# zju-vipa/ProtoPFormer

Measured on AMD Instinct MI355X. Metric: images/sec train step, deit_small+2000 protos, bs256, 1/2/4/8 MI355X, higher is better.
Workload: dtype bf16; 1 GPU; deit_small_patch16_224, synthetic 224x224, 2000x384 prototypes, 200 classes, k=81, batch 256/GPU (BASELINE.json configs[2]), train step = fwd+CE+PPC+bwd+allreduce+AdamW+EMA, DropPath 0.1; blocks after the token reservation run compacted on the 1+k reserved rows (equal to the masked full-length blocks to bf16 rounding); bf16 backbone: the reserved tokens differ from the fp32 reference's in ~2-3 % o; global_batch=256, parallelism=dp1

## Files before the change

### include/ppf_hip.h

```cpp
#ifndef PPF_HIP_H
#define PPF_HIP_H

#include <stddef.h>
#include <stdint.h>

#ifdef __cplusplus
extern "C" {
#endif

typedef struct ihipStream_t* ppf_stream_t;

#define PPF_ERR_SHAPE (-1)
#define PPF_ERR_ALIGN (-2)
#define PPF_ERR_ARG (-3)

#define PPF_ABI_VERSION 10

const char* ppf_last_error(void);
int ppf_abi_version(void);
int ppf_device_info(int* cu_count, int* clock_mhz, char* name, int name_len);
int ppf_stream_arm(ppf_stream_t stream, int on);
int ppf_stream_wait_stream(ppf_stream_t dst, ppf_stream_t src);
int64_t ppf_stream_mark(ppf_stream_t stream);
int ppf_stream_wait_mark(ppf_stream_t stream, int64_t ticket);
// ... 159 lines not shown
                        ppf_stream_t stream);
int ppf_assemble_tokens_bwd(const float* dx, void* dtok, float* dpos, float* dcls, int B, int Np, int D, int lead,
                            ppf_stream_t stream);
int ppf_sigmoid_bwd_blocks(int rows);
int ppf_sigmoid_bwd(const float* df, const float* f, void* dz, float* dbias, int rows, int cols, float* partial, size_t partial_bytes,
                    ppf_stream_t stream);
int ppf_adamw_step(float* p, const float* g, float* m, float* v, float* ema, void* p16, int64_t n, int nseg,
                   const int64_t* seg_bounds, const float* seg_lr, const float* seg_wd, float beta1, float beta2, float eps,
                   int step, float ema_decay, float grad_scale, ppf_stream_t stream);
int ppf_adamw_step_dev(float* p, const float* g, float* m, float* v, float* ema, void* p16, int64_t n, int nseg,
                       const int64_t* seg_bounds, const float* hyper, float beta1, float beta2, float eps, float ema_decay,
                       ppf_stream_t stream);
int ppf_adamw_step_guarded(float* p, const float* g, float* m, float* v, float* ema, void* p16, int64_t n, int nseg,
                           const int64_t* seg_bounds, const float* hyper, float beta1, float beta2, float eps, float ema_decay,
                           const float* loss, int* nonfinite_flag, ppf_stream_t stream);
int ppf_hyper_set(float* hyper, const float* host_vals, int n, ppf_stream_t stream);
int ppf_clip_grad_blocks(void);
int ppf_clip_grad_scale(const float* g, int64_t n, float max_norm, float pre_scale, float* partial, float* hyper, float* norm_out,
                        ppf_stream_t stream);
int ppf_droppath_scales(float* out, const float* keep, int nslot, int B, uint64_t seed, void* state_u64, ppf_stream_t stream);
int ppf_reserved_rows_map(const int* idx, int* rows, int B, int k, int N, ppf_stream_t stream);
int ppf_gather_rows(const void* src, const int* rows, void* dst, int nrows, int row_bytes, ppf_stream_t stream);
int ppf_scatter_rows(const void* src, const int* rows, void* dst, int nrows_src, int nrows_dst, int row_bytes, ppf_stream_t stream);
int ppf_memset_zero(void* ptr, size_t bytes, ppf_stream_t stream);
int ppf_copy_2d(void* dst, int64_t dst_pitch, const void* src, int64_t src_pitch, int64_t width, int64_t rows, ppf_stream_t stream);
int ppf_image_finish_u8(const void* in_u8_hwc, float* out_nchw, int B, int H, int W, const float* mean3, const float* std3,
                        const int* rects, uint64_t seed, const void* state_u64, ppf_stream_t stream);
#define PPF_MIX_KIND 0
#define PPF_MIX_YL 1
#define PPF_MIX_YH 2
#define PPF_MIX_XL 3
#define PPF_MIX_XH 4
#define PPF_MIX_WSELF 5
#define PPF_MIX_WOTHER 6
#define PPF_MIX_WORDS 8
int ppf_mixup_apply(float* x, const int* table_host, int* table_dev, int B, int Cc, int H, int W, ppf_stream_t stream);
int ppf_mixup_target(const void* label_i64, const float* lam, int lam_stride, float off_value, float on_value, float* target, int B,
                     int C, ppf_stream_t stream);
int ppf_scale_by_scalar(const float* x, const float* scalar_dev, float* out, int64_t n, ppf_stream_t stream);

int ppf_im2col_patch_f32(const float* img, float* cols, int B, int C, int H, int W, int patch, ppf_stream_t stream);
int ppf_layernorm_fwd_f32(const float* x, const int* row_map, const float* w, const float* b, float* y, int rows, int D, float eps,
                          ppf_stream_t stream);
int ppf_epilogue_f32(float* C, const float* bias, int kind, const float* res, const float* rowscale, int rows_per_group,
                     const float* colscale, int M, int N, ppf_stream_t stream);
int ppf_attn_fwd_f32(const float* qkv, float* out, const float* policy, float* headmean, int NP, int B, int H, int N, int D,
// ... 11 lines not shown
```

### protopformer_amd/backbone.py

```python
import functools
import os

import torch
import torch.nn as nn

from . import _lib, ops
from .ops import EPI_ATOMIC, EPI_BF16, EPI_DGELU, EPI_F32, EPI_GELU, EPI_RESID, EPI_SIGMOID_F32

LN_EPS = 1e-6
_KEEP_CACHE = {}
_ROW_BWD_MAX_ELEMS = 12_000_000


def _row_bwd(M, D):
    return M * D <= _ROW_BWD_MAX_ELEMS


def droppath_scales(rates, B, device, training):
    slots = [r if training else 0.0 for r in rates]
    active = [i for i, r in enumerate(slots) if r > 0.0]
    if not active:
        return None, [-1] * len(slots)
    key = (tuple(slots), str(device))
    st = _KEEP_CACHE.get(key)
# ... 391 lines not shown
    dnf = head_bwd(ppnet, store, saved, df)
    alloc = ops.zeros if head["row_map"] is not None else (lambda shape, dtype, device: torch.empty(shape, dtype=dtype, device=device))
    dx = alloc((M, D), torch.float32, dev)
    dyb = lane.track(alloc((M, D), torch.bfloat16, dev))
    last = feats.blocks[-1]
    lnb(dnf, x_last.reshape(M, D), feats.norm.weight, head["meanf"], head["rstdf"], store.grad_view(feats.norm.weight),
        store.grad_view(feats.norm.bias), dx_out=dx, row_map=head["row_map"], cast_out=dyb, rowscale=layers[-1]["s2"],
        rows_per_group=N, dbias_next=store.grad_view(last.mlp.fc2.bias))
    gs = getattr(ppnet, "_grad_sync", None)
    if gs is not None:
        chunk_ready(gs, lane, gs.tail_chunk)
    bwd = functools.partial(block_bwd, next_dyb=dyb_ring(lane, D), lnb=lnb, dgrad=functools.partial(_dgrad, store),
                            attn_bwd=lambda blk, L, dao: ops.attn_bwd(L["qkv"], L["ao"], dao, L["rowmax"], L["zinv"], B, feats.num_heads, L["N"], D,
                                                                      policy=L["policy"], self_keep=True, eps_n=L["eps_n"]))
    bias_done = True
    for i in range(len(layers) - 1, -1, -1):
        L = layers[i]
        Nl = L["N"]
        row_tile = row_tile_bwd(store, feats.blocks[i], D, ops.rowgemm_tile_rows(B * Nl, Nl, backward=True)) if _row_bwd(B * Nl, D) else None
        dyb, bias_done = bwd(feats.blocks[i], store, L, dx, dyb, bias_done, (feats.blocks[i - 1], layers[i - 1]) if i > 0 else None,
                             row_tile=row_tile)
        if i > 0 and L["rows"] is not None:
            Mf = B * layers[i - 1]["N"]
            dx = ops.scatter_rows(dx, L["rows"], Mf)
            dyb = lane.track(ops.scatter_rows(dyb, L["rows"], Mf))
        if gs is not None and i in gs.block_chunk:
            chunk_ready(gs, lane, gs.block_chunk[i])
    if layers and layers[0]["rows"] is not None:
        dx = ops.scatter_rows(dx, layers[0]["rows"], B * (feats.patch_embed.num_patches + 1))
    return embed_bwd(ppnet, store, saved, dx, 1)


class TokensFn(torch.autograd.Function):

    @staticmethod
    def forward(ctx, img, ppnet, dp, *params):
        store = ppnet.flat_store()
        store.refresh_bf16()
        feats = ppnet.features
        need_bwd = any(ctx.needs_input_grad)
        if need_bwd and "t16_params" in ppnet._arch_fns:
            if store._t16 is None:
                store.register_transposed(ppnet._arch_fns["t16_params"](feats))
            if store._t16 is not None and not store._t16["fresh"] and feats.embed_dim <= 256:
                wgrad_lane(store).submit(store.refresh_t16, (store.bf16, store._t16["buf"]), defer=True)
            else:
                store.refresh_t16()
        saved = {} if need_bwd else None
        (layer, k), = ppnet.reserve_layer_nums
        fwd = ppnet._arch_fns
        x = fwd["embed"](feats, store, img, saved)
        x_out, cls_attn, idx, layers = fwd["blocks"](feats, store, x, layer, k, dp, save=need_bwd)
# ... 27 lines not shown
```

### protopformer_amd/csrc/elementwise.hip

```cpp
#include "ppf_common.h"
#include "ppf_hip.h"

namespace {

__global__ __launch_bounds__(256) void cast_kernel(const float* __restrict__ in, bf16_t* __restrict__ out, int64_t n8) {
    for (int64_t i = (int64_t)blockIdx.x * 256 + threadIdx.x; i < n8; i += (int64_t)gridDim.x * 256) {
        const float4 a = reinterpret_cast<const float4*>(in)[2 * i], b = reinterpret_cast<const float4*>(in)[2 * i + 1];
        reinterpret_cast<uint4*>(out)[i] = make_uint4(pack_bf16x2(a.x, a.y), pack_bf16x2(a.z, a.w), pack_bf16x2(b.x, b.y), pack_bf16x2(b.z, b.w));
    }
}

__global__ __launch_bounds__(256) void widen_kernel(const bf16_t* __restrict__ in, float* __restrict__ out, int64_t n8) {
    for (int64_t i = (int64_t)blockIdx.x * 256 + threadIdx.x; i < n8; i += (int64_t)gridDim.x * 256) {
        const uint4 u = reinterpret_cast<const uint4*>(in)[i];
        const float2 a = unpack_bf16x2(u.x), b = unpack_bf16x2(u.y), c = unpack_bf16x2(u.z), d = unpack_bf16x2(u.w);
        reinterpret_cast<float4*>(out)[2 * i] = make_float4(a.x, a.y, b.x, b.y);
        reinterpret_cast<float4*>(out)[2 * i + 1] = make_float4(c.x, c.y, d.x, d.y);
    }
}

__global__ __launch_bounds__(256) void im2col_kernel(const float* __restrict__ img, bf16_t* __restrict__ cols, int B, int C,
                                                     int H, int W, int p, int64_t total8) {
    const int gh = H / p, gw = W / p, pp8 = p / 8, kdim = C * p * p;
    for (int64_t i = (int64_t)blockIdx.x * 256 + threadIdx.x; i < total8; i += (int64_t)gridDim.x * 256) {
// ... 192 lines not shown
                out[i] = floorf(kp + u) / kp;
            }
        }
    }
    __syncthreads();
    if (threadIdx.x == 0) state[0] = step + 1;
}

__global__ __launch_bounds__(256) void rows_map_kernel(const int* __restrict__ idx, int* __restrict__ rows, int B, int k, int N) {
    const int i = blockIdx.x * 256 + threadIdx.x;
    if (i >= B * (k + 1)) return;
    const int b = i / (k + 1), j = i % (k + 1);
    rows[i] = b * N + (j == 0 ? 0 : 1 + idx[b * k + j - 1]);
}
__global__ __launch_bounds__(256) void move_rows_kernel(const uint4* __restrict__ src, const int* __restrict__ rows, uint4* __restrict__ dst,
                                                        int nrows, int vec, int scatter) {
    const int64_t total = (int64_t)nrows * vec;
    for (int64_t i = (int64_t)blockIdx.x * 256 + threadIdx.x; i < total; i += (int64_t)gridDim.x * 256) {
        const int r = (int)(i / vec), c = (int)(i % vec);
        const int64_t o = (int64_t)rows[r] * vec + c;
        if (scatter) dst[o] = src[i]; else dst[i] = src[o];
    }
}
__global__ __launch_bounds__(256) void scale_by_kernel(const float* __restrict__ x, const float* __restrict__ scalar, float* __restrict__ out, int64_t n) {
    const float s = *scalar;
    for (int64_t i = (int64_t)blockIdx.x * 256 + threadIdx.x; i < n; i += (int64_t)gridDim.x * 256) out[i] = x[i] * s;
}

struct FinishParams { const unsigned char* in; float* out; const int* rects; int B, H, W; float mean[3], inv_std[3]; uint64_t seed; const unsigned long long* state; };
__global__ __launch_bounds__(256) void image_finish_kernel(const FinishParams p) {
    const int64_t hw = (int64_t)p.H * p.W, total4 = (int64_t)p.B * hw / 4;
    const unsigned long long step = p.state ? p.state[0] : 0ull;
    for (int64_t i = (int64_t)blockIdx.x * 256 + threadIdx.x; i < total4; i += (int64_t)gridDim.x * 256) {
        const int b = (int)((i * 4) / hw);
        const int64_t pix = i * 4 - (int64_t)b * hw;
        const int y = (int)(pix / p.W), x = (int)(pix % p.W);
        const unsigned char* src = p.in + ((int64_t)b * hw + pix) * 3;
        const uint32_t w0 = reinterpret_cast<const uint32_t*>(src)[0], w1 = reinterpret_cast<const uint32_t*>(src)[1], w2 = reinterpret_cast<const uint32_t*>(src)[2];
        const unsigned char px[12] = {(unsigned char)w0, (unsigned char)(w0 >> 8), (unsigned char)(w0 >> 16), (unsigned char)(w0 >> 24),
                                      (unsigned char)w1, (unsigned char)(w1 >> 8), (unsigned char)(w1 >> 16), (unsigned char)(w1 >> 24),
                                      (unsigned char)w2, (unsigned char)(w2 >> 8), (unsigned char)(w2 >> 16), (unsigned char)(w2 >> 24)};
        int ry = 0, rx = 0, rh = 0, rw = 0;
        if (p.rects) { ry = p.rects[4 * b]; rx = p.rects[4 * b + 1]; rh = p.rects[4 * b + 2]; rw = p.rects[4 * b + 3]; }
        const bool row_in = rh > 0 && y >= ry && y < ry + rh;
#pragma unroll
        for (int c = 0; c < 3; ++c) {
// ... 170 lines not shown
    PPF_CHECK_ARG(nslot > 0 && B > 0 && out && keep && state_u64, PPF_ERR_ARG, "ppf_droppath_scales: bad arguments");
    return ppf_launch<droppath_kernel>(dim3(1), dim3(256), 0, stream, "ppf_droppath_scales", out, keep, nslot, B, seed, (unsigned long long*)state_u64);
}

int ppf_reserved_rows_map(const int* idx, int* rows, int B, int k, int N, hipStream_t stream) {
    PPF_CHECK_ARG(B > 0 && k > 0 && N > k, PPF_ERR_SHAPE, "ppf_reserved_rows_map: bad shape B=%d k=%d N=%d", B, k, N);
    return ppf_launch<rows_map_kernel>(dim3((B * (k + 1) + 255) / 256), dim3(256), 0, stream, "ppf_reserved_rows_map", idx, rows, B, k, N);
}

int ppf_gather_rows(const void* src, const int* rows, void* dst, int nrows, int row_bytes, hipStream_t stream) {
    PPF_CHECK_ARG(nrows > 0 && row_bytes > 0 && row_bytes % 16 == 0, PPF_ERR_ALIGN, "ppf_gather_rows: row_bytes=%d must be a positive multiple of 16", row_bytes);
    return ppf_launch<move_rows_kernel>(dim3(grid_for((int64_t)nrows * (row_bytes / 16))), dim3(256), 0, stream, "ppf_gather_rows", (const uint4*)src, rows,
                                        (uint4*)dst, nrows, row_bytes / 16, 0);
}

int ppf_scatter_rows(const void* src, const int* rows, void* dst, int nrows_src, int nrows_dst, int row_bytes, hipStream_t stream) {
    PPF_CHECK_ARG(nrows_src > 0 && nrows_dst >= nrows_src && row_bytes > 0 && row_bytes % 16 == 0, PPF_ERR_ALIGN, "ppf_scatter_rows: bad arguments");
    hipError_t e = ppf_memset_async(dst, 0, (size_t)nrows_dst * row_bytes, stream);
    if (e != hipSuccess) { ppf_set_error("ppf_scatter_rows: memset failed: %s", hipGetErrorString(e)); return (int)e; }
    return ppf_launch<move_rows_kernel>(dim3(grid_for((int64_t)nrows_src * (row_bytes / 16))), dim3(256), 0, stream, "ppf_scatter_rows", (const uint4*)src, rows,
                                        (uint4*)dst, nrows_src, row_bytes / 16, 1);
}

int ppf_image_finish_u8(const void* in_u8_hwc, float* out_nchw, int B, int H, int W, const float* mean3, const float* std3, const int* rects,
                        uint64_t seed, const void* state_u64, hipStream_t stream) {
    PPF_CHECK_ARG(B > 0 && H > 0 && W > 0 && W % 4 == 0 && in_u8_hwc && out_nchw && mean3 && std3, PPF_ERR_ARG, "ppf_image_finish_u8: bad arguments (W %% 4 == 0)");
    PPF_CHECK_ARG((((uintptr_t)in_u8_hwc) & 3) == 0 && (((uintptr_t)out_nchw) & 15) == 0, PPF_ERR_ALIGN, "ppf_image_finish_u8: alignment");
    FinishParams p;
    p.in = (const unsigned char*)in_u8_hwc; p.out = out_nchw; p.rects = rects; p.B = B; p.H = H; p.W = W; p.seed = seed;
    p.state = (const unsigned long long*)state_u64;
    for (int c = 0; c < 3; ++c) { p.mean[c] = mean3[c]; p.inv_std[c] = 1.0f / std3[c]; }
    return ppf_launch<image_finish_kernel>(dim3(grid_for((int64_t)B * H * W / 4)), dim3(256), 0, stream, "ppf_image_finish_u8", p);
}

int ppf_memset_zero(void* ptr, size_t bytes, hipStream_t stream) {
    if (bytes == 0) return 0;
    hipError_t e = ppf_memset_async(ptr, 0, bytes, stream);
    if (e != hipSuccess) { ppf_set_error("ppf_memset_zero: %s", hipGetErrorString(e)); return (int)e; }
    return 0;
}

int ppf_scale_by_scalar(const float* x, const float* scalar_dev, float* out, int64_t n, hipStream_t stream) {
    PPF_CHECK_ARG(n > 0 && x && scalar_dev && out, PPF_ERR_ARG, "ppf_scale_by_scalar: bad arguments");
    return ppf_launch<scale_by_kernel>(dim3(grid_for(n)), dim3(256), 0, stream, "ppf_scale_by_scalar", x, scalar_dev, out, n);
}

// ... 19 lines not shown
```

### protopformer_amd/csrc/head.hip

```cpp
#include "ppf_common.h"
#include "ppf_hip.h"
#include "ppf_select.h"

namespace {

constexpr int MAXPPC = 16;

struct PpcParams {
    const float* act;
    const int* idx;
    const long long* label;
    int B, P, T, ppc, side;
    float cov_thresh, mean_thresh;
    float* partial;
    float* gcov;
    float* gmean;
};

__global__ __launch_bounds__(256) void ppc_kernel(const PpcParams p) {
    __shared__ float mu[MAXPPC][2], S[MAXPPC], hinge_cov[MAXPPC], gmu[MAXPPC][2];
    __shared__ float mean_sum;
    const int lane = threadIdx.x & 63, wave = threadIdx.x >> 6, b = blockIdx.x;
    const int N = p.side * p.side;
    const float nfac = (float)N / (float)(N - 1);
    const int lab = (int)p.label[b];
    const float inv_cnt = 1.0f / ((float)p.B * (float)p.ppc);
    for (int j = wave; j < p.ppc; j += 4) {
        const float* w = p.act + ((size_t)b * p.P + (size_t)lab * p.ppc + j) * p.T;
        float s = 0.f, sx = 0.f, sy = 0.f;
        for (int t = lane; t < p.T; t += 64) {
            const int id = p.idx[(size_t)b * p.T + t];
            const float wt = w[t], x = (float)(id / p.side), y = (float)(id % p.side);
            s += wt; sx += wt * x; sy += wt * y;
        }
        s = wave_sum(s); sx = wave_sum(sx); sy = wave_sum(sy);
        const float mx = sx / s, my = sy / s;
        float v = 0.f;
        for (int t = lane; t < p.T; t += 64) {
            const int id = p.idx[(size_t)b * p.T + t];
            const float dx = (float)(id / p.side) - mx, dy = (float)(id % p.side) - my;
            v += w[t] * (dx * dx + dy * dy);
        }
        v = wave_sum(v) / s;
        const float c = 0.5f * nfac * v;
        const bool on = c > p.cov_thresh;
        for (int t = lane; t < p.T; t += 64) {
            const int id = p.idx[(size_t)b * p.T + t];
            const float dx = (float)(id / p.side) - mx, dy = (float)(id % p.side) - my;
            p.gcov[((size_t)b * p.ppc + j) * p.T + t] = on ? inv_cnt * 0.5f * nfac * ((dx * dx + dy * dy) - v) / s : 0.f;
        }
        if (lane == 0) { mu[j][0] = mx; mu[j][1] = my; S[j] = s; hinge_cov[j] = on ? c - p.cov_thresh : 0.f; }
    }
    __syncthreads();
    if (threadIdx.x == 0) {
        float ms = 0.f;
        for (int j = 0; j < p.ppc; ++j) { gmu[j][0] = 0.f; gmu[j][1] = 0.f; }
        const float pair_norm = 1.0f / ((float)p.B * (float)p.ppc * (float)p.ppc);
        for (int j = 0; j < p.ppc; ++j)
            for (int k = 0; k < p.ppc; ++k) {
                if (j == k) continue;
                const float dx = mu[j][0] - mu[k][0], dy = mu[j][1] - mu[k][1];
                const float d = sqrtf(dx * dx + dy * dy);
                if (p.mean_thresh - d > 0.f) {
                    ms += p.mean_thresh - d;
                    if (d > 0.f) {
                        gmu[j][0] -= 2.0f * pair_norm * dx / d;
                        gmu[j][1] -= 2.0f * pair_norm * dy / d;
                    }
                }
            }
        mean_sum = ms;
        float cs = 0.f;
        for (int j = 0; j < p.ppc; ++j) cs += hinge_cov[j];
        p.partial[2 * b] = cs;
        p.partial[2 * b + 1] = ms;
    }
    __syncthreads();
    for (int j = wave; j < p.ppc; j += 4) {
        const float mx = mu[j][0], my = mu[j][1], s = S[j], gx = gmu[j][0], gy = gmu[j][1];
        for (int t = lane; t < p.T; t += 64) {
            const int id = p.idx[(size_t)b * p.T + t];
            const float dx = (float)(id / p.side) - mx, dy = (float)(id % p.side) - my;
            p.gmean[((size_t)b * p.ppc + j) * p.T + t] = (gx * dx + gy * dy) / s;
        }
    }
}

__global__ __launch_bounds__(256) void reduce_cols_kernel(const float* in, int n, int stride, int cols, float s0, float s1, float* out) {
    __shared__ float red[256];
    for (int c = 0; c < cols; ++c) {
        float s = 0.f;
        for (int i = threadIdx.x; i < n; i += 256) s += in[(size_t)i * stride + c];
        red[threadIdx.x] = s;
        __syncthreads();
        for (int o = 128; o > 0; o >>= 1) {
            if (threadIdx.x < o) red[threadIdx.x] += red[threadIdx.x + o];
            __syncthreads();
        }
        if (threadIdx.x == 0) out[c] = red[0] * (c == 0 ? s0 : s1);
        __syncthreads();
    }
}

__global__ __launch_bounds__(256) void ppc_bwd_kernel(const float* gcov, const float* gmean, const float* up_cov, const float* up_mean,
                                                      const long long* label, float* g_full, int B, int P, int T, int ppc) {
    const int b = blockIdx.x;
    const float uc = up_cov ? up_cov[0] : 0.f, um = up_mean ? up_mean[0] : 0.f;
    const int lab = (int)label[b];
    for (int i = threadIdx.x; i < ppc * T; i += 256) {
        const int j = i / T, t = i % T;
        g_full[((size_t)b * P + (size_t)lab * ppc + j) * T + t] = uc * gcov[((size_t)b * ppc + j) * T + t] + um * gmean[((size_t)b * ppc + j) * T + t];
    }
}

__global__ __launch_bounds__(256) void ce_kernel(const float* logits, const long long* label, float* per_sample, float* dlogits, int B, int C) {
    const int lane = threadIdx.x & 63, wave = threadIdx.x >> 6;
    const int b = blockIdx.x * 4 + wave;
    if (b >= B) return;
    const float* row = logits + (size_t)b * C;
    float mx = -INFINITY;
    for (int c = lane; c < C; c += 64) mx = fmaxf(mx, row[c]);
    mx = wave_max(mx);
    float s = 0.f;
    for (int c = lane; c < C; c += 64) s += __expf(row[c] - mx);
    s = wave_sum(s);
    const int lab = (int)label[b];
    const float lse = mx + __logf(s);
    if (lane == 0) per_sample[b] = lse - row[lab];
    const float invB = 1.0f / (float)B;
    for (int c = lane; c < C; c += 64) dlogits[(size_t)b * C + c] = (__expf(row[c] - lse) - (c == lab ? 1.0f : 0.0f)) * invB;
}

__global__ __launch_bounds__(256) void soft_ce_kernel(const float* logits, const float* target, const long long* label, float smoothing,
                                                      float* per_sample, float* dlogits, int B, int C) {
    const int lane = threadIdx.x & 63, wave = threadIdx.x >> 6;
    const int b = blockIdx.x * 4 + wave;
    if (b >= B) return;
    const float* row = logits + (size_t)b * C;
    float mxf = -INFINITY;
    for (int c = lane; c < C; c += 64) mxf = fmaxf(mxf, row[c]);
    const double mx = (double)wave_max(mxf);
    double s = 0.0;
    for (int c = lane; c < C; c += 64) s += exp((double)row[c] - mx);
    const double ls = log(wave_sum_f64(s));
    const double invB = 1.0 / (double)B;
    if (target) {
        const float* t = target + (size_t)b * C;
        double st = 0.0, acc = 0.0;
        for (int c = lane; c < C; c += 64) {
            const double tc = (double)t[c];
            st += tc;
            acc += tc * ((mx - (double)row[c]) + ls);
        }
        st = wave_sum_f64(st);
        acc = wave_sum_f64(acc);
        if (lane == 0) per_sample[b] = (float)acc;
        for (int c = lane; c < C; c += 64)
            dlogits[(size_t)b * C + c] = (float)((exp((double)row[c] - mx - ls) * st - (double)t[c]) * invB);
    } else {
        const long long lab = label[b];
        double dlab = 0.0, dsum = 0.0;
        for (int c = lane; c < C; c += 64) {
            const double d = mx - (double)row[c];
            dsum += d;
            if (c == lab) dlab = d;
        }
        dlab = wave_sum_f64(dlab);
        dsum = wave_sum_f64(dsum);
        const double sm = (double)smoothing, conf = 1.0 - sm, off = sm / (double)C;
        if (lane == 0) per_sample[b] = (float)(conf * (dlab + ls) + sm * (dsum / (double)C + ls));
        for (int c = lane; c < C; c += 64)
            dlogits[(size_t)b * C + c] = (float)((exp((double)row[c] - mx - ls) - (c == lab ? conf : 0.0) - off) * invB);
    }
}

constexpr int EVAL_MAX_WG = 1024, EVAL_NV = 6;
__device__ double g_eval_partial[EVAL_MAX_WG * EVAL_NV];

__device__ __forceinline__ int wave_argmax_first(const float* row, int C, int lane, float& mx_out) {
    float mx = -INFINITY;
    int at = 0x7fffffff;
    for (int c = lane; c < C; c += 64) {
        const float x = row[c];
        if (x > mx || at == 0x7fffffff) { mx = x; at = c; }
    }
    wave_first(mx, at);
    mx_out = mx;
    return at;
}

__global__ __launch_bounds__(256) void eval_metrics_kernel(const float* __restrict__ logits, const float* __restrict__ logits_global,
                                                           const float* __restrict__ logits_local, const long long* __restrict__ label,
                                                           int B, int C) {
    __shared__ double red[4][EVAL_NV];
    const int lane = threadIdx.x & 63, wave = threadIdx.x >> 6;
    double ce = 0.0;
// ... 213 lines not shown
    float p0 = 0.f, p1 = 0.f;
    if (n < q0.N) { for (int z = 0; z < q0.S; ++z) p0 += part[q0.part_off + ((size_t)z * M + m) * q0.N + n]; if (q0.out) q0.out[(size_t)m * q0.ldo + n] = q0.alpha * p0; }
    if (n < q1.N) { for (int z = 0; z < q1.S; ++z) p1 += part[q1.part_off + ((size_t)z * M + m) * q1.N + n]; if (q1.out) q1.out[(size_t)m * q1.ldo + n] = q1.alpha * p1; }
    if (sum) sum[(size_t)m * ldsum + n] = q0.c * p0 + q1.c * p1;
}

__global__ __launch_bounds__(256) void axpbypcz_kernel(const float* x, const float* y, const float* z, float* out, float a, float b, float c, int64_t n) {
    for (int64_t i = (int64_t)blockIdx.x * 256 + threadIdx.x; i < n; i += (int64_t)gridDim.x * 256) out[i] = a * x[i] + b * y[i] + c * z[i];
}
__global__ __launch_bounds__(256) void axpby_kernel(const float* x, const float* y, float* out, float a, float b, int64_t n) {
    for (int64_t i = (int64_t)blockIdx.x * 256 + threadIdx.x; i < n; i += (int64_t)gridDim.x * 256) out[i] = a * x[i] + b * y[i];
}

}

extern "C" {

int ppf_ppc_loss(const float* act, const int* idx, const void* label, int B, int P, int T, int ppc, int side, float cov_thresh,
                 float mean_thresh, float* partial, float* gcov, float* gmean, float* loss, hipStream_t stream) {
    PPF_CHECK_ARG(B > 0 && P > 0 && T > 0 && ppc >= 1 && ppc <= MAXPPC && side >= 2 && P % ppc == 0, PPF_ERR_SHAPE, "ppf_ppc_loss: bad shape");
    PpcParams p;
    p.act = act; p.idx = idx; p.label = (const long long*)label; p.B = B; p.P = P; p.T = T; p.ppc = ppc; p.side = side;
    p.cov_thresh = cov_thresh; p.mean_thresh = mean_thresh; p.partial = partial; p.gcov = gcov; p.gmean = gmean;
    if (int rc = ppf_launch<ppc_kernel>(dim3(B), dim3(256), 0, stream, "ppf_ppc_loss", p)) return rc;
    return ppf_launch<reduce_cols_kernel>(dim3(1), dim3(256), 0, stream, "ppf_ppc_loss", partial, B, 2, 2, 1.0f / ((float)B * ppc), 1.0f / ((float)B * ppc * ppc), loss);
}

int ppf_ppc_loss_bwd(const float* gcov, const float* gmean, const float* up_cov, const float* up_mean, const void* label, float* g_full, int B,
                     int P, int T, int ppc, hipStream_t stream) {
    PPF_CHECK_ARG(B > 0 && P > 0 && T > 0 && ppc >= 1, PPF_ERR_SHAPE, "ppf_ppc_loss_bwd: bad shape");
    return ppf_launch<ppc_bwd_kernel>(dim3(B), dim3(256), 0, stream, "ppf_ppc_loss_bwd", gcov, gmean, up_cov, up_mean, (const long long*)label, g_full, B, P, T, ppc);
}

int ppf_cross_entropy(const float* logits, const void* label, float* per_sample, float* dlogits, float* loss, int B, int C, hipStream_t stream) {
    PPF_CHECK_ARG(B > 0 && C > 0, PPF_ERR_SHAPE, "ppf_cross_entropy: bad shape");
    if (int rc = ppf_launch<ce_kernel>(dim3((B + 3) / 4), dim3(256), 0, stream, "ppf_cross_entropy", logits, (const long long*)label, per_sample, dlogits, B, C)) return rc;
    return ppf_launch<reduce_cols_kernel>(dim3(1), dim3(256), 0, stream, "ppf_cross_entropy", per_sample, B, 1, 1, 1.0f / (float)B, 0.f, loss);
}

int ppf_soft_cross_entropy(const float* logits, const float* target, const void* label, float smoothing, float* per_sample, float* dlogits,
                           float* loss, int B, int C, hipStream_t stream) {
    PPF_CHECK_ARG(B > 0 && C > 0, PPF_ERR_SHAPE, "ppf_soft_cross_entropy: bad shape B=%d C=%d", B, C);
    PPF_CHECK_ARG(logits && per_sample && dlogits && loss, PPF_ERR_ARG, "ppf_soft_cross_entropy: null pointer");
    PPF_CHECK_ARG((target == nullptr) != (label == nullptr), PPF_ERR_ARG, "ppf_soft_cross_entropy: pass exactly one of target / label");
    PPF_CHECK_ARG(target || (smoothing >= 0.f && smoothing <= 1.f), PPF_ERR_ARG, "ppf_soft_cross_entropy: smoothing %g outside [0, 1]",
                  (double)smoothing);
    if (int rc = ppf_launch<soft_ce_kernel>(dim3((B + 3) / 4), dim3(256), 0, stream, "ppf_soft_cross_entropy", logits, target, (const long long*)label, smoothing,
                                            per_sample, dlogits, B, C)) return rc;
    return ppf_launch<reduce_cols_kernel>(dim3(1), dim3(256), 0, stream, "ppf_soft_cross_entropy", per_sample, B, 1, 1, 1.0f / (float)B, 0.f, loss);
}

int ppf_eval_metrics(const float* logits, const float* logits_global, const float* logits_local, const void* label, double* acc, int B, int C,
                     hipStream_t stream) {
    PPF_CHECK_ARG(B > 0 && C > 0, PPF_ERR_SHAPE, "ppf_eval_metrics: bad shape B=%d C=%d", B, C);
    PPF_CHECK_ARG(logits && label && acc, PPF_ERR_ARG, "ppf_eval_metrics: null pointer");
    const int nwg = (B + 3) / 4 < EVAL_MAX_WG ? (B + 3) / 4 : EVAL_MAX_WG;
    if (int rc = ppf_launch<eval_metrics_kernel>(dim3(nwg), dim3(256), 0, stream, "ppf_eval_metrics", logits, logits_global, logits_local, (const long long*)label, B, C)) return rc;
    return ppf_launch<eval_metrics_finish_kernel>(dim3(1), dim3(256), 0, stream, "ppf_eval_metrics", acc, nwg, B, logits_global != nullptr, logits_local != nullptr);
}

int ppf_sgemm(const float* A, const float* Bm, float* C, int M, int N, int K, int64_t sam, int64_t sak, int64_t sbn, int64_t sbk, int ldc,
              float alpha, float beta, float* workspace, int64_t workspace_floats, hipStream_t stream) {
    PPF_CHECK_ARG(M > 0 && N > 0 && K > 0, PPF_ERR_SHAPE, "ppf_sgemm: bad shape");
    int S = workspace ? (int)(workspace_floats / ((int64_t)M * N)) : 1;
    if (S > 16) S = 16;
    if (S > (K + 127) / 128) S = (K + 127) / 128;
    if (S < 1) S = 1;
    const int kchunk = ((K + S - 1) / S + 31) / 32 * 32;
    S = (K + kchunk - 1) / kchunk;
    int rc;
    if ((int64_t)M * N * K >= (int64_t(1) << 28) && M >= 64 && N >= 64) {
        const int tiles = ((N + SM_T - 1) / SM_T) * ((M + SM_T - 1) / SM_T);
// ... 50 lines not shown
```

### protopformer_amd/csrc/ppf_runtime.hip

```cpp
#include "ppf_common.h"
#include "ppf_hip.h"
#include <cstdarg>
#include <cstdio>
#include <cstdlib>

static thread_local char g_err[512] = "";

extern "C" {

void ppf_set_error(const char* fmt, ...) {
    va_list ap;
    va_start(ap, fmt);
    vsnprintf(g_err, sizeof(g_err), fmt, ap);
    va_end(ap);
}

const char* ppf_last_error(void) { return g_err; }

int ppf_abi_version(void) { return PPF_ABI_VERSION; }

int ppf_device_info(int* cu_count, int* clock_mhz, char* name, int name_len) {
    hipDeviceProp_t prop;
    int dev = 0;
    hipError_t e = hipGetDevice(&dev);
// ... 61 lines not shown
    hipError_t e = hipStreamWaitEvent(stream, ring_event(ticket), 0);
    if (e != hipSuccess) { ppf_set_error("ppf_stream_wait_mark: %s", hipGetErrorString(e)); return (int)e; }
    return 0;
}

namespace {
PpfEventPool g_path[PPF_PROBE_NTAGS];
constexpr size_t PATH_PROBE_CAP = 4096;
bool g_path_on = false;
}

}

hipEvent_t ppf_take_stop_event(hipStream_t s) {
    for (auto& a : g_arm)
        if (a.used && a.armed && a.s == s) { a.ev = ring_event(g_seq++); a.have = true; return a.ev; }
    return nullptr;
}
void ppf_note_enqueue(hipStream_t s) {
    for (auto& a : g_arm)
        if (a.used && a.s == s) a.have = false;
}

int ppf_cu_count() {
    static const int cus = [] {
        int dev = 0, n = 256;
        (void)hipGetDevice(&dev);
        (void)hipDeviceGetAttribute(&n, hipDeviceAttributeMultiprocessorCount, dev);
        return n > 0 ? n : 256;
    }();
    return cus;
}

std::pair<hipEvent_t, hipEvent_t> PpfEventPool::acquire() {
    if (used == pool.size()) {
        hipEvent_t a = nullptr, b = nullptr;
        (void)hipEventCreateWithFlags(&a, hipEventDisableSystemFence); (void)hipEventCreateWithFlags(&b, hipEventDisableSystemFence);
        pool.emplace_back(a, b);
    }
    return pool[used++];
}
void PpfEventPool::reset() { used = 0; flops = 0.0; bytes = 0.0; }
void PpfEventPool::destroy() {
    for (auto& e : pool) { (void)hipEventDestroy(e.first); (void)hipEventDestroy(e.second); }
    pool.clear(); used = 0;
}
// ... 47 lines not shown
```

### protopformer_amd/ops.py

```python
import torch

from . import _lib

EPI_BF16, EPI_F32, EPI_GELU, EPI_SIGMOID_F32, EPI_RESID, EPI_DGELU, EPI_ATOMIC = range(7)


DOMINANT_NAME = ("weight-gradient bf16 MFMA GEMM, split over the contraction, ordered partial tiles: wgrad8_kernel<4,2> / <2,4> (256x128 / 128x256 tiles) "
                 "and gemm_kernel<TA=1,TB=1,EPI_PARTIAL,COLSUM> (128x128)")


_WORKSPACE = {}
_GEMM_WS = {}
_RETIRED_WS = []


def _workspace(device, nbytes, pool=_WORKSPACE):
    key = (device, _lib.stream_ptr())
    buf = pool.get(key)
    if buf is None or buf.numel() < nbytes:
        if buf is not None:
            _RETIRED_WS.append(buf)
        buf = torch.empty(max(nbytes, 64 << 20), dtype=torch.uint8, device=device)
        pool[key] = buf
    return buf
# ... 845 lines not shown
def cat_rows(first, rest):
    B, N, D = rest.shape
    out = torch.empty((B, N + 1, D), dtype=rest.dtype, device=rest.device)
    o2 = out.reshape(B, (N + 1) * D)
    copy_2d(o2[:, :D], first.reshape(B, D))
    copy_2d(o2[:, D:], rest.reshape(B, N * D))
    return out


def reserved_rows_map(idx, N):
    B, k = idx.shape
    rows = torch.empty(B * (k + 1), dtype=torch.int32, device=idx.device)
    _lib.call("ppf_reserved_rows_map", idx, rows, B, k, N)
    return rows


def gather_rows(src, rows):
    _chk(src)
    dst = torch.empty((rows.numel(), src.shape[1]), dtype=src.dtype, device=src.device)
    _lib.call("ppf_gather_rows", src, rows, dst, rows.numel(), src.shape[1] * src.element_size())
    return dst


def scatter_rows(src, rows, nrows_dst):
    _chk(src)
    dst = torch.empty((nrows_dst, src.shape[1]), dtype=src.dtype, device=src.device)
    _lib.call("ppf_scatter_rows", src, rows, dst, src.shape[0], nrows_dst, src.shape[1] * src.element_size())
    return dst


def droppath_draw(out, keep, seed, state):
    nslot, B = out.shape
    _lib.call("ppf_droppath_scales", out, keep, nslot, B, int(seed) & 0xFFFFFFFFFFFFFFFF, state)
    return out


def scale_by_scalar(x, scalar):
    out = torch.empty_like(x)
    _lib.call("ppf_scale_by_scalar", x, scalar, out, x.numel())
    return out


def th_fused_ok(H, N, D):
    return bool(_lib.lib().ppf_th_fused_supported(H, N, D))


def th_fwd(qkv, wl, bl, ww, bw, hm_out, B, H, N, D):
    NP, NPK = (N + 3) // 4 * 4, (N + 7) // 8 * 8
    a16 = torch.empty((B, H, N, NPK), dtype=torch.bfloat16, device=qkv.device)
    rowmax = torch.empty((B, H, N), dtype=torch.float32, device=qkv.device)
# ... 159 lines not shown
```

Baseline: 17320 images/sec.

## Fuse loss reductions into kernels via last-block finish; grouped row scatter

The cross-entropy, soft cross-entropy and PPC loss kernels now do their own final reduction. The last workgroup to arrive on a per-stream atomic counter reduces the partials, which removes the separate one-block reduce_cols launch after each. The PPC kernel also moves to 1024 threads. Backward row scatter switches to a per-sample grouped kernel that builds an inverse map in LDS and writes each destination row once, copied or zeroed, with nontemporal stores. This is meant to avoid a separate zero-fill-plus-scatter pass. The cost is atomic counter state tied to a stream slot table, and reliance on correct fence ordering.

```diff
diff --git a/include/ppf_hip.h b/include/ppf_hip.h
--- a/include/ppf_hip.h
+++ b/include/ppf_hip.h
@@ -205,6 +205,8 @@
 int ppf_reserved_rows_map(const int* idx, int* rows, int B, int k, int N, ppf_stream_t stream);
 int ppf_gather_rows(const void* src, const int* rows, void* dst, int nrows, int row_bytes, ppf_stream_t stream);
 int ppf_scatter_rows(const void* src, const int* rows, void* dst, int nrows_src, int nrows_dst, int row_bytes, ppf_stream_t stream);
+int ppf_scatter_rows_grouped(const void* src, const int* rows, void* dst, int groups, int rows_per_group_src, int rows_per_group_dst,
+                             int row_bytes, ppf_stream_t stream);
 int ppf_memset_zero(void* ptr, size_t bytes, ppf_stream_t stream);
 int ppf_copy_2d(void* dst, int64_t dst_pitch, const void* src, int64_t src_pitch, int64_t width, int64_t rows, ppf_stream_t stream);
 int ppf_image_finish_u8(const void* in_u8_hwc, float* out_nchw, int B, int H, int W, const float* mean3, const float* std3,
diff --git a/protopformer_amd/backbone.py b/protopformer_amd/backbone.py
--- a/protopformer_amd/backbone.py
+++ b/protopformer_amd/backbone.py
@@ -437,12 +437,12 @@
                              row_tile=row_tile)
         if i > 0 and L["rows"] is not None:
             Mf = B * layers[i - 1]["N"]
-            dx = ops.scatter_rows(dx, L["rows"], Mf)
-            dyb = lane.track(ops.scatter_rows(dyb, L["rows"], Mf))
+            dx = ops.scatter_rows(dx, L["rows"], Mf, groups=B)
+            dyb = lane.track(ops.scatter_rows(dyb, L["rows"], Mf, groups=B))
         if gs is not None and i in gs.block_chunk:
             chunk_ready(gs, lane, gs.block_chunk[i])
     if layers and layers[0]["rows"] is not None:
-        dx = ops.scatter_rows(dx, layers[0]["rows"], B * (feats.patch_embed.num_patches + 1))
+        dx = ops.scatter_rows(dx, layers[0]["rows"], B * (feats.patch_embed.num_patches + 1), groups=B)
     return embed_bwd(ppnet, store, saved, dx, 1)
 
 
diff --git a/protopformer_amd/csrc/elementwise.hip b/protopformer_amd/csrc/elementwise.hip
--- a/protopformer_amd/csrc/elementwise.hip
+++ b/protopformer_amd/csrc/elementwise.hip
@@ -238,6 +238,32 @@
         if (scatter) dst[o] = src[i]; else dst[i] = src[o];
     }
 }
+__global__ __launch_bounds__(256) void scatter_rows_grouped_kernel(const uint4* __restrict__ src, const int* __restrict__ rows, uint4* __restrict__ dst,
+                                                                   int ns, int nd, int vec) {
+    extern __shared__ int inv[];
+    const int b = blockIdx.x;
+    for (int d = threadIdx.x; d < nd; d += 256) inv[d] = -1;
+    __syncthreads();
+    for (int j = threadIdx.x; j < ns; j += 256) {
+        const int d = rows[(size_t)b * ns + j] - b * nd;
+        if (d >= 0 && d < nd) inv[d] = j;
+    }
+    __syncthreads();
+    typedef unsigned int u32x4 __attribute__((ext_vector_type(4)));
+    const int per = (nd + gridDim.y - 1) / gridDim.y, d0 = blockIdx.y * per, d1 = min(nd, d0 + per);
+    const int lane = threadIdx.x & 63;
+    for (int d = d0 + (threadIdx.x >> 6); d < d1; d += 4) {
+        const int j = inv[d];
+        u32x4* o = reinterpret_cast<u32x4*>(dst + ((size_t)b * nd + d) * vec);
+        if (j >= 0) {
+            const u32x4* s = reinterpret_cast<const u32x4*>(src + ((size_t)b * ns + j) * vec);
+            for (int c = lane; c < vec; c += 64) __builtin_nontemporal_store(s[c], o + c);
+        } else {
+            const u32x4 zero = {0u, 0u, 0u, 0u};
+            for (int c = lane; c < vec; c += 64) __builtin_nontemporal_store(zero, o + c);
+        }
+    }
+}
 __global__ __launch_bounds__(256) void scale_by_kernel(const float* __restrict__ x, const float* __restrict__ scalar, float* __restrict__ out, int64_t n) {
     const float s = *scalar;
     for (int64_t i = (int64_t)blockIdx.x * 256 + threadIdx.x; i < n; i += (int64_t)gridDim.x * 256) out[i] = x[i] * s;
@@ -454,6 +480,22 @@
                                         (uint4*)dst, nrows_src, row_bytes / 16, 1);
 }
 
+int ppf_scatter_rows_grouped(const void* src, const int* rows, void* dst, int groups, int rows_per_group_src, int rows_per_group_dst, int row_bytes,
+                             hipStream_t stream) {
+    PPF_CHECK_ARG(src && rows && dst && groups > 0 && rows_per_group_src > 0 && rows_per_group_dst >= rows_per_group_src, PPF_ERR_SHAPE,
+                  "ppf_scatter_rows_grouped: bad shape groups=%d rows %d -> %d", groups, rows_per_group_src, rows_per_group_dst);
+    PPF_CHECK_ARG(row_bytes > 0 && row_bytes % 16 == 0 && ((uintptr_t)src & 15) == 0 && ((uintptr_t)dst & 15) == 0, PPF_ERR_ALIGN,
+                  "ppf_scatter_rows_grouped: row_bytes=%d and both pointers must be multiples of 16", row_bytes);
+    PPF_CHECK_ARG(rows_per_group_dst <= 16000 && groups <= 0x7fffffff / rows_per_group_dst,
+                  PPF_ERR_SHAPE, "ppf_scatter_rows_grouped: group of %d rows too large (inverse table in LDS: <= 16000 rows)", rows_per_group_dst);
+    int split = (8 * ppf_cu_count() + groups - 1) / groups;
+    if (split > rows_per_group_dst) split = rows_per_group_dst;
+    if (split > 65535) split = 65535;
+    if (split < 1) split = 1;
+    return ppf_launch<scatter_rows_grouped_kernel>(dim3(groups, split), dim3(256), (size_t)rows_per_group_dst * sizeof(int), stream, "ppf_scatter_rows_grouped",
+                                                   (const uint4*)src, rows, (uint4*)dst, rows_per_group_src, rows_per_group_dst, row_bytes / 16);
+}
+
 int ppf_image_finish_u8(const void* in_u8_hwc, float* out_nchw, int B, int H, int W, const float* mean3, const float* std3, const int* rects,
                         uint64_t seed, const void* state_u64, hipStream_t stream) {
     PPF_CHECK_ARG(B > 0 && H > 0 && W > 0 && W % 4 == 0 && in_u8_hwc && out_nchw && mean3 && std3, PPF_ERR_ARG, "ppf_image_finish_u8: bad arguments (W %% 4 == 0)");
diff --git a/protopformer_amd/csrc/head.hip b/protopformer_amd/csrc/head.hip
--- a/protopformer_amd/csrc/head.hip
+++ b/protopformer_amd/csrc/head.hip
@@ -1,4 +1,5 @@
 #include "ppf_common.h"
+#include "ppf_finish.h"
 #include "ppf_hip.h"
 #include "ppf_select.h"
 
@@ -15,17 +16,42 @@
     float* partial;
     float* gcov;
     float* gmean;
+    float* loss;
+    float s_cov, s_mean;
+    int slot;
 };
 
-__global__ __launch_bounds__(256) void ppc_kernel(const PpcParams p) {
+enum { FIN_CE = 0, FIN_SOFT_CE = 1, FIN_PPC = 2, FIN_SCALARS = 4 };
+__device__ unsigned g_fin_scalar[PPF_FINISH_STREAMS][FIN_SCALARS];
+
+__device__ __forceinline__ void reduce_cols(float* red, const float* in, int n, int stride, int cols, float s0, float s1, float* out) {
+    for (int c = 0; c < cols; ++c) {
+        if (threadIdx.x < 256) {
+            float s = 0.f;
+            for (int i = threadIdx.x; i < n; i += 256) s += in[(size_t)i * stride + c];
+            red[threadIdx.x] = s;
+        }
+        __syncthreads();
+        for (int o = 128; o > 0; o >>= 1) {
+            if (threadIdx.x < o) red[threadIdx.x] += red[threadIdx.x + o];
+            __syncthreads();
+        }
+        if (threadIdx.x == 0) out[c] = red[0] * (c == 0 ? s0 : s1);
+        __syncthreads();
+    }
+}
+
+constexpr int PPC_THREADS = 1024;
+__global__ __launch_bounds__(PPC_THREADS) void ppc_kernel(const PpcParams p) {
     __shared__ float mu[MAXPPC][2], S[MAXPPC], hinge_cov[MAXPPC], gmu[MAXPPC][2];
     __shared__ float mean_sum;
+    __shared__ float red[256];
     const int lane = threadIdx.x & 63, wave = threadIdx.x >> 6, b = blockIdx.x;
     const int N = p.side * p.side;
     const float nfac = (float)N / (float)(N - 1);
     const int lab = (int)p.label[b];
     const float inv_cnt = 1.0f / ((float)p.B * (float)p.ppc);
-    for (int j = wave; j < p.ppc; j += 4) {
+    for (int j = wave; j < p.ppc; j += PPC_THREADS / 64) {
         const float* w = p.act + ((size_t)b * p.P + (size_t)lab * p.ppc + j) * p.T;
         float s = 0.f, sx = 0.f, sy = 0.f;
         for (int t = lane; t < p.T; t += 64) {
@@ -72,11 +98,11 @@
         mean_sum = ms;
         float cs = 0.f;
         for (int j = 0; j < p.ppc; ++j) cs += hinge_cov[j];
-        p.partial[2 * b] = cs;
-        p.partial[2 * b + 1] = ms;
+        ppf_finish_store(p.partial + 2 * b, cs);
+        ppf_finish_store(p.partial + 2 * b + 1, ms);
     }
     __syncthreads();
-    for (int j = wave; j < p.ppc; j += 4) {
+    for (int j = wave; j < p.ppc; j += PPC_THREADS / 64) {
         const float mx = mu[j][0], my = mu[j][1], s = S[j], gx = gmu[j][0], gy = gmu[j][1];
         for (int t = lane; t < p.T; t += 64) {
             const int id = p.idx[(size_t)b * p.T + t];
@@ -84,22 +110,8 @@
             p.gmean[((size_t)b * p.ppc + j) * p.T + t] = (gx * dx + gy * dy) / s;
         }
     }
-}
-
-__global__ __launch_bounds__(256) void reduce_cols_kernel(const float* in, int n, int stride, int cols, float s0, float s1, float* out) {
-    __shared__ float red[256];
-    for (int c = 0; c < cols; ++c) {
-        float s = 0.f;
-        for (int i = threadIdx.x; i < n; i += 256) s += in[(size_t)i * stride + c];
-        red[threadIdx.x] = s;
-        __syncthreads();
-        for (int o = 128; o > 0; o >>= 1) {
-            if (threadIdx.x < o) red[threadIdx.x] += red[threadIdx.x + o];
-            __syncthreads();
-        }
-        if (threadIdx.x == 0) out[c] = red[0] * (c == 0 ? s0 : s1);
-        __syncthreads();
-    }
+    if (ppf_finish_arrive(&g_fin_scalar[p.slot][FIN_PPC], gridDim.x, reinterpret_cast<unsigned*>(red)))
+        reduce_cols(red, p.partial, p.B, 2, 2, p.s_cov, p.s_mean, p.loss);
 }
 
 __global__ __launch_bounds__(256) void ppc_bwd_kernel(const float* gcov, const float* gmean, const float* up_cov, const float* up_mean,
@@ -113,29 +125,31 @@
     }
 }
 
-__global__ __launch_bounds__(256) void ce_kernel(const float* logits, const long long* label, float* per_sample, float* dlogits, int B, int C) {
+__global__ __launch_bounds__(256) void ce_kernel(const float* logits, const long long* label, float* per_sample, float* dlogits, float* loss,
+                                                 int B, int C, int slot) {
+    __shared__ float red[256];
     const int lane = threadIdx.x & 63, wave = threadIdx.x >> 6;
     const int b = blockIdx.x * 4 + wave;
-    if (b >= B) return;
-    const float* row = logits + (size_t)b * C;
-    float mx = -INFINITY;
-    for (int c = lane; c < C; c += 64) mx = fmaxf(mx, row[c]);
-    mx = wave_max(mx);
-    float s = 0.f;
-    for (int c = lane; c < C; c += 64) s += __expf(row[c] - mx);
-    s = wave_sum(s);
-    const int lab = (int)label[b];
-    const float lse = mx + __logf(s);
-    if (lane == 0) per_sample[b] = lse - row[lab];
-    const float invB = 1.0f / (float)B;
-    for (int c = lane; c < C; c += 64) dlogits[(size_t)b * C + c] = (__expf(row[c] - lse) - (c == lab ? 1.0f : 0.0f)) * invB;
-}
-
-__global__ __launch_bounds__(256) void soft_ce_kernel(const float* logits, const float* target, const long long* label, float smoothing,
-                                                      float* per_sample, float* dlogits, int B, int C) {
-    const int lane = threadIdx.x & 63, wave = threadIdx.x >> 6;
-    const int b = blockIdx.x * 4 + wave;
-    if (b >= B) return;
+    if (b < B) {
+        const float* row = logits + (size_t)b * C;
+        float mx = -INFINITY;
+        for (int c = lane; c < C; c += 64) mx = fmaxf(mx, row[c]);
+        mx = wave_max(mx);
+        float s = 0.f;
+        for (int c = lane; c < C; c += 64) s += __expf(row[c] - mx);
+        s = wave_sum(s);
+        const int lab = (int)label[b];
+        const float lse = mx + __logf(s);
+        if (lane == 0) ppf_finish_store(per_sample + b, lse - row[lab]);
+        const float invB = 1.0f / (float)B;
+        for (int c = lane; c < C; c += 64) dlogits[(size_t)b * C + c] = (__expf(row[c] - lse) - (c == lab ? 1.0f : 0.0f)) * invB;
+    }
+    if (ppf_finish_arrive(&g_fin_scalar[slot][FIN_CE], gridDim.x, reinterpret_cast<unsigned*>(red)))
+        reduce_cols(red, per_sample, B, 1, 1, 1.0f / (float)B, 0.f, loss);
+}
+
+__device__ __forceinline__ void soft_ce_row(const float* logits, const float* target, const long long* label, float smoothing, float* per_sample,
+                                            float* dlogits, int B, int C, int b, int lane) {
     const float* row = logits + (size_t)b * C;
     float mxf = -INFINITY;
     for (int c = lane; c < C; c += 64) mxf = fmaxf(mxf, row[c]);
@@ -154,7 +168,7 @@
         }
         st = wave_sum_f64(st);
         acc = wave_sum_f64(acc);
-        if (lane == 0) per_sample[b] = (float)acc;
+        if (lane == 0) ppf_finish_store(per_sample + b, (float)acc);
         for (int c = lane; c < C; c += 64)
             dlogits[(size_t)b * C + c] = (float)((exp((double)row[c] - mx - ls) * st - (double)t[c]) * invB);
     } else {
@@ -168,10 +182,19 @@
         dlab = wave_sum_f64(dlab);
         dsum = wave_sum_f64(dsum);
         const double sm = (double)smoothing, conf = 1.0 - sm, off = sm / (double)C;
-        if (lane == 0) per_sample[b] = (float)(conf * (dlab + ls) + sm * (dsum / (double)C + ls));
+        if (lane == 0) ppf_finish_store(per_sample + b, (float)(conf * (dlab + ls) + sm * (dsum / (double)C + ls)));
         for (int c = lane; c < C; c += 64)
             dlogits[(size_t)b * C + c] = (float)((exp((double)row[c] - mx - ls) - (c == lab ? conf : 0.0) - off) * invB);
     }
+}
+__global__ __launch_bounds__(256) void soft_ce_kernel(const float* logits, const float* target, const long long* label, float smoothing,
+                                                      float* per_sample, float* dlogits, float* loss, int B, int C, int slot) {
+    __shared__ float red[256];
+    const int lane = threadIdx.x & 63, wave = threadIdx.x >> 6;
+    const int b = blockIdx.x * 4 + wave;
+    if (b < B) soft_ce_row(logits, target, label, smoothing, per_sample, dlogits, B, C, b, lane);
+    if (ppf_finish_arrive(&g_fin_scalar[slot][FIN_SOFT_CE], gridDim.x, reinterpret_cast<unsigned*>(red)))
+        reduce_cols(red, per_sample, B, 1, 1, 1.0f / (float)B, 0.f, loss);
 }
 
 constexpr int EVAL_MAX_WG = 1024, EVAL_NV = 6;
@@ -431,8 +454,9 @@
     PpcParams p;
     p.act = act; p.idx = idx; p.label = (const long long*)label; p.B = B; p.P = P; p.T = T; p.ppc = ppc; p.side = side;
     p.cov_thresh = cov_thresh; p.mean_thresh = mean_thresh; p.partial = partial; p.gcov = gcov; p.gmean = gmean;
-    if (int rc = ppf_launch<ppc_kernel>(dim3(B), dim3(256), 0, stream, "ppf_ppc_loss", p)) return rc;
-    return ppf_launch<reduce_cols_kernel>(dim3(1), dim3(256), 0, stream, "ppf_ppc_loss", partial, B, 2, 2, 1.0f / ((float)B * ppc), 1.0f / ((float)B * ppc * ppc), loss);
+    p.loss = loss; p.s_cov = 1.0f / ((float)B * ppc); p.s_mean = 1.0f / ((float)B * ppc * ppc);
+    if ((p.slot = ppf_finish_slot(stream, "ppf_ppc_loss")) < 0) return PPF_ERR_ARG;
+    return ppf_launch<ppc_kernel>(dim3(B), dim3(PPC_THREADS), 0, stream, "ppf_ppc_loss", p);
 }
 
 int ppf_ppc_loss_bwd(const float* gcov, const float* gmean, const float* up_cov, const float* up_mean, const void* label, float* g_full, int B,
@@ -443,8 +467,9 @@
 
 int ppf_cross_entropy(const float* logits, const void* label, float* per_sample, float* dlogits, float* loss, int B, int C, hipStream_t stream) {
     PPF_CHECK_ARG(B > 0 && C > 0, PPF_ERR_SHAPE, "ppf_cross_entropy: bad shape");
-    if (int rc = ppf_launch<ce_kernel>(dim3((B + 3) / 4), dim3(256), 0, stream, "ppf_cross_entropy", logits, (const long long*)label, per_sample, dlogits, B, C)) return rc;
-    return ppf_launch<reduce_cols_kernel>(dim3(1), dim3(256), 0, stream, "ppf_cross_entropy", per_sample, B, 1, 1, 1.0f / (float)B, 0.f, loss);
+    const int slot = ppf_finish_slot(stream, "ppf_cross_entropy");
+    if (slot < 0) return PPF_ERR_ARG;
+    return ppf_launch<ce_kernel>(dim3((B + 3) / 4), dim3(256), 0, stream, "ppf_cross_entropy", logits, (const long long*)label, per_sample, dlogits, loss, B, C, slot);
 }
 
 int ppf_soft_cross_entropy(const float* logits, const float* target, const void* label, float smoothing, float* per_sample, float* dlogits,
@@ -454,9 +479,10 @@
     PPF_CHECK_ARG((target == nullptr) != (label == nullptr), PPF_ERR_ARG, "ppf_soft_cross_entropy: pass exactly one of target / label");
     PPF_CHECK_ARG(target || (smoothing >= 0.f && smoothing <= 1.f), PPF_ERR_ARG, "ppf_soft_cross_entropy: smoothing %g outside [0, 1]",
                   (double)smoothing);
-    if (int rc = ppf_launch<soft_ce_kernel>(dim3((B + 3) / 4), dim3(256), 0, stream, "ppf_soft_cross_entropy", logits, target, (const long long*)label, smoothing,
-                                            per_sample, dlogits, B, C)) return rc;
-    return ppf_launch<reduce_cols_kernel>(dim3(1), dim3(256), 0, stream, "ppf_soft_cross_entropy", per_sample, B, 1, 1, 1.0f / (float)B, 0.f, loss);
+    const int slot = ppf_finish_slot(stream, "ppf_soft_cross_entropy");
+    if (slot < 0) return PPF_ERR_ARG;
+    return ppf_launch<soft_ce_kernel>(dim3((B + 3) / 4), dim3(256), 0, stream, "ppf_soft_cross_entropy", logits, target, (const long long*)label, smoothing,
+                                      per_sample, dlogits, loss, B, C, slot);
 }
 
 int ppf_eval_metrics(const float* logits, const float* logits_global, const float* logits_local, const void* label, double* acc, int B, int C,
diff --git a/protopformer_amd/csrc/ppf_finish.h b/protopformer_amd/csrc/ppf_finish.h
--- /dev/null
+++ b/protopformer_amd/csrc/ppf_finish.h
@@ -0,0 +1,27 @@
+#pragma once
+#include "ppf_common.h"
+
+constexpr int PPF_FINISH_STREAMS = 64;
+
+__attribute__((visibility("hidden"))) int ppf_finish_slot(hipStream_t stream, const char* who);
+
+__device__ __forceinline__ void ppf_finish_store(float* p, float v) { __hip_atomic_store(p, v, __ATOMIC_RELAXED, __HIP_MEMORY_SCOPE_AGENT); }
+
+__device__ __forceinline__ bool ppf_finish_arrive(unsigned* counter, unsigned n, unsigned* lds_word) {
+    asm volatile("s_waitcnt vmcnt(0)" ::: "memory");
+    __syncthreads();
+    if (threadIdx.x == 0) {
+        const unsigned old = __hip_atomic_fetch_add(counter, 1u, __ATOMIC_RELAXED, __HIP_MEMORY_SCOPE_AGENT);
+        const bool last = old + 1u == n;
+        if (last) {
+            __hip_atomic_store(counter, 0u, __ATOMIC_RELAXED, __HIP_MEMORY_SCOPE_AGENT);
+            __builtin_amdgcn_fence(__ATOMIC_ACQUIRE, "agent");
+            asm volatile("s_waitcnt vmcnt(0)" ::: "memory");
+        }
+        *lds_word = last ? 1u : 0u;
+    }
+    __syncthreads();
+    const bool mine = *lds_word != 0u;
+    __syncthreads();
+    return mine;
+}
diff --git a/protopformer_amd/csrc/ppf_runtime.hip b/protopformer_amd/csrc/ppf_runtime.hip
--- a/protopformer_amd/csrc/ppf_runtime.hip
+++ b/protopformer_amd/csrc/ppf_runtime.hip
@@ -1,4 +1,5 @@
 #include "ppf_common.h"
+#include "ppf_finish.h"
 #include "ppf_hip.h"
 #include <cstdarg>
 #include <cstdio>
@@ -107,6 +108,19 @@
         if (a.used && a.s == s) a.have = false;
 }
 
+int ppf_finish_slot(hipStream_t stream, const char* who) {
+    static hipStream_t table[PPF_FINISH_STREAMS];
+    static int used = 0;
+    for (int i = 0; i < used; ++i)
+        if (table[i] == stream) return i;
+    if (used == PPF_FINISH_STREAMS) {
+        ppf_set_error("%s: more than %d streams have used the in-launch reductions of this process", who, PPF_FINISH_STREAMS);
+        return -1;
+    }
+    table[used] = stream;
+    return used++;
+}
+
 int ppf_cu_count() {
     static const int cus = [] {
         int dev = 0, n = 256;
diff --git a/protopformer_amd/ops.py b/protopformer_amd/ops.py
--- a/protopformer_amd/ops.py
+++ b/protopformer_amd/ops.py
@@ -891,10 +891,14 @@
     return dst
 
 
-def scatter_rows(src, rows, nrows_dst):
+def scatter_rows(src, rows, nrows_dst, groups=None):
     _chk(src)
     dst = torch.empty((nrows_dst, src.shape[1]), dtype=src.dtype, device=src.device)
-    _lib.call("ppf_scatter_rows", src, rows, dst, src.shape[0], nrows_dst, src.shape[1] * src.element_size())
+    if groups is None:
+        _lib.call("ppf_scatter_rows", src, rows, dst, src.shape[0], nrows_dst, src.shape[1] * src.element_size())
+    else:
+        assert src.shape[0] % groups == 0 and nrows_dst % groups == 0
+        _lib.call("ppf_scatter_rows_grouped", src, rows, dst, groups, src.shape[0] // groups, nrows_dst // groups, src.shape[1] * src.element_size())
     return dst
 
 
```

Measured after the change: 17340 images/sec (median of 4 runs). About the same (+0.1%).
